# Ensembl/WiggleTools

Measured on AMD Instinct MI355X. Metric: genomic bp/s (whole node) for 'mean' over N BigWig tracks, higher is better.
Workload: dtype f64

## Files before the change

### wiggletools_amd/csrc/wt_delta.h

```cpp
#ifndef WT_DELTA_H_
#define WT_DELTA_H_

#define WT_DELTA_K 8
#define WT_DELTA_GROUP 16
#ifndef WT_DELTA_PARK
#define WT_DELTA_PARK 1
#endif
#ifndef WT_DELTA_U
#define WT_DELTA_U 4
#endif
#define WT_DELTA_TILE (64 * WT_DELTA_U)
#ifndef WT_DELTA_COPY2
#define WT_DELTA_COPY2 1
#endif
#ifndef WT_DELTA_ONE_TILE
#define WT_DELTA_ONE_TILE 1
#endif
#define WT_DELTA_TF 2048
#define WT_MAX_DELTA_T 1024
#define WT_DELTA_SQ_T0 768

struct WtDeltaShared {
    long long base_v;
    int32_t base_c;
    int32_t emin, emax, bad;
    unsigned long long base_qa, base_qb;
    long long base_v1;
    unsigned long long base_qa1, base_qb1;
    int32_t base_c1, risk;
};

#define WT_DELTA_QSHIFT 40

struct WtDeltaCtx {
    long long *acc;
    uint32_t *ev;
    long long *ltv;
    int32_t *ltc;
    long long *gtv;
    int32_t *gtc;
    long long *tbase;
    uint32_t *tpfx;
    uint16_t *tfirst;
    uint32_t *tdef;
    unsigned long long *qa, *qb;
    unsigned long long *ltqa, *ltqb;
    unsigned long long *gtqa, *gtqb;
    WtDeltaShared *dsh;
    int32_t np;
};

struct WtDeltaLane {
    long long pv[WT_DELTA_K];
    int32_t pc[WT_DELTA_K];
    uint32_t evmask;
    long long tv;
    int32_t tc;
    long long wv;
    int32_t wc;
    unsigned long long tqa, tqb;
    unsigned long long wqa, wqb;
};

WT_DEV void wt_delta_ctx_init(WtDeltaCtx &d, const WtParams &P, char *lds) {
    d.acc = (long long *) (lds + P.off_acc);
    d.ev = (uint32_t *) (lds + P.off_ev);
    d.ltv = (long long *) (lds + P.off_ltv);
    d.ltc = (int32_t *) (lds + P.off_ltc);
    d.gtv = (long long *) (lds + P.off_gtv);
    d.gtc = (int32_t *) (lds + P.off_gtc);
    d.tbase = (long long *) (lds + P.off_tbase);
    d.tpfx = (uint32_t *) (lds + P.off_tpfx);
    d.tfirst = (uint16_t *) (lds + P.off_tfirst);
    d.tdef = (uint32_t *) (lds + P.off_tdef);
    const int ns = P.delta_ns > 1 ? P.delta_ns : 1;
    d.np = ns * P.W;
    d.qa = (unsigned long long *) (lds + P.off_qa);
    d.qb = d.qa + d.np;
    d.ltqa = (unsigned long long *) (lds + P.off_ltq);
    d.ltqb = d.ltqa + ns * (P.W / WT_DELTA_K);
    d.gtqa = (unsigned long long *) (lds + P.off_gtq);
    d.gtqb = d.gtqa + ns * (P.W / WT_DELTA_K / WT_DELTA_GROUP);
    d.dsh = (WtDeltaShared *) (lds + P.off_dsh);
}

#ifdef WT_EMU
WT_DEV void wt_lds_add32(uint32_t *p, uint32_t v) { *p += v; }
WT_DEV void wt_lds_addi32(int32_t *p, int32_t v) { *p += v; }
WT_DEV void wt_lds_max32(int32_t *p, int32_t v) { if (v > *p) *p = v; }
#else
WT_DEV void wt_lds_add32(uint32_t *p, uint32_t v) { atomicAdd((unsigned int *) p, (unsigned int) v); }
WT_DEV void wt_lds_addi32(int32_t *p, int32_t v) { atomicAdd(p, v); }
WT_DEV void wt_lds_max32(int32_t *p, int32_t v) { atomicMax(p, v); }
#endif

WT_DEV int wt_delta_max_span(int n_tracks) {
    int lg = 0;
    while ((1ll << lg) < (long long) n_tracks) lg++;
    return 29 - lg;
}

template <bool QQ = false, bool TT = false>
WT_DEV void wt_delta_zero(const WtParams &P, WtCtx &c, WtDeltaCtx &d, int tid, int nt) {
    const int np = TT ? 2 * P.W : P.W;
    for (int x = tid; x < np; x += nt) { d.acc[x] = 0; d.ev[x] = 0; }
    if constexpr (QQ)
        for (int x = tid; x < np; x += nt) { d.qa[x] = 0; d.qb[x] = 0; }
    if (tid == 0) {
        d.dsh->base_v = 0; d.dsh->base_c = 0;
        if constexpr (QQ) { d.dsh->base_qa = 0; d.dsh->base_qb = 0; }
        if constexpr (TT) { d.dsh->base_v1 = 0; d.dsh->base_c1 = 0; d.dsh->base_qa1 = 0; d.dsh->base_qb1 = 0; d.dsh->risk = 0; }
        d.dsh->emin = P.def_emin; d.dsh->emax = P.def_emax; d.dsh->bad = 0;
// ... 899 lines not shown
        const unsigned higher = k + 1 < WT_DELTA_K ? um >> (k + 1) : 0u;
        const uint32_t fin_rel = higher ? (uint32_t) (p0 + k + 1 + wt_ctz64((uint64_t) higher)) : after_rel;
        sv[WT_STAGE_AT(idx)] = L.res[k];
        sp[WT_STAGE_AT(idx)] = (uint32_t) (p0 + k) | (fin_rel << 16);
        idx++;
    }
}

#ifndef WT_EMU
template <int OP>
WT_DEV void wt_delta_stage_ep(const WtParams &P, WtCtx &c, WtDeltaCtx &d, const WtLane<WT_DELTA_K> &L, unsigned em, unsigned um, unsigned idx, int tid, int nt) {
    const int per = nt / WT_BAD_SUB;
    if (c.sh->bad_slot >= 0 && tid % per == 0) c.epfx[32 + tid / per] = idx;
    if (!em) return;
    const int p0 = tid * WT_DELTA_K;
    const int32_t after = wt_next_breakpoint(P, c, p0 + WT_DELTA_K - 1);
    const int32_t w0 = c.sh->w0;
    const uint32_t after_rel = after < c.sh->w1 ? (uint32_t) (after - w0) : WT_DELTA_FAR;
    double *sv = (double *) d.acc;
    uint32_t *sp = d.ev;
#pragma unroll
    for (int k = 0; k < WT_DELTA_K; k++) {
        if (!((em >> k) & 1u)) continue;
        const unsigned higher = k + 1 < WT_DELTA_K ? um >> (k + 1) : 0u;
        const uint32_t fin_rel = higher ? (uint32_t) (p0 + k + 1 + wt_ctz64((uint64_t) higher)) : after_rel;
        sv[WT_STAGE_AT(idx)] = L.res[k];
        sp[WT_STAGE_AT(idx)] = (uint32_t) (p0 + k) | (fin_rel << 16);
        idx++;
    }
}
WT_DEV void wt_delta_note_offset_ep(const WtParams &P, WtCtx &c, int lane) {
    if (c.sh->bad_slot >= 0 && P.bad_goff && lane < WT_BAD_SUB)
        P.bad_goff[(long long) c.sh->bad_slot * WT_BAD_SUB + lane] = c.sh->goffset + (long long) c.epfx[32 + lane];
}
#endif

WT_DEV void wt_delta_copy_out(const WtParams &P, WtCtx &c, WtDeltaCtx &d, int tid, int nt) {
    const int n = c.sh->n_emit;
    const long long goff = c.sh->goffset;
    const int32_t w0 = c.sh->w0, far = c.sh->next_bp;
    const double *sv = (const double *) d.acc;
    const uint32_t *sp = d.ev;
    unsigned long long bp = 0;
#if !defined(WT_EMU) && WT_DELTA_COPY2
    struct __attribute__((packed, aligned(4))) I2 { int32_t x[2]; };
    struct __attribute__((packed, aligned(8))) D2 { double x[2]; };
    for (int i = 2 * tid; i < n; i += 2 * nt) {
        const unsigned a0 = WT_STAGE_AT((unsigned) i);
        const bool two = i + 1 < n;
        const uint32_t pf0 = sp[a0], pf1 = two ? sp[a0 + 1] : 0u;
        const double v0 = sv[a0], v1 = two ? sv[a0 + 1] : 0.0;
        const int32_t st0 = w0 + (int32_t) (pf0 & 0xffffu), st1 = w0 + (int32_t) (pf1 & 0xffffu);
        const int32_t fin0 = (pf0 >> 16) == WT_DELTA_FAR ? far : w0 + (int32_t) (pf0 >> 16);
        const int32_t fin1 = (pf1 >> 16) == WT_DELTA_FAR ? far : w0 + (int32_t) (pf1 >> 16);
        bp += (unsigned long long) (fin0 - st0) + (two ? (unsigned long long) (fin1 - st1) : 0ull);
        const long long o = goff + i;
        if (two && o + 1 < P.capacity) {
            I2 s2, f2; D2 d2;
            s2.x[0] = st0; s2.x[1] = st1; f2.x[0] = fin0; f2.x[1] = fin1; d2.x[0] = v0; d2.x[1] = v1;
            *(I2 *) (P.o_start + o) = s2;
            *(I2 *) (P.o_finish + o) = f2;
            *(D2 *) (P.o_value + o) = d2;
        } else if (o < P.capacity) {
            P.o_start[o] = st0; P.o_finish[o] = fin0; P.o_value[o] = v0;
        }
    }
#else
    for (int i = tid; i < n; i += nt) {
        const uint32_t pf = sp[WT_STAGE_AT((unsigned) i)];
        const int32_t st = w0 + (int32_t) (pf & 0xffffu);
        const int32_t fin = (pf >> 16) == WT_DELTA_FAR ? far : w0 + (int32_t) (pf >> 16);
        bp += (unsigned long long) (fin - st);
        const long long o = goff + i;
        if (o >= P.capacity) continue;
        P.o_start[o] = st;
        P.o_finish[o] = fin;
        P.o_value[o] = sv[WT_STAGE_AT((unsigned) i)];
    }
#endif
    bp = wt_wave_sum_u64(bp);
    if (bp && wt_wave_leader(tid & 63)) wt_lds_add64(&c.sh->bp_sum, bp);
}

WT_DEV void wt_delta_nextw(const WtParams &P, WtCtx &c, int tid, int nt) {
    for (int w = nt - 1 - tid; w < P.n_words; w += nt) {
        int x = w + 1;
        while (x < P.n_words && c.U[x] == 0) x++;
        c.nextw[w] = (int16_t) (x < P.n_words ? x : -1);
    }
}


#ifndef WT_EMU
WT_DEV unsigned wt_wave_scan_u32(unsigned v, int lane) {
    return wt_wave_scan32(v, 0u, [](uint32_t a, uint32_t b) { return a + b; });
}
WT_DEV long long wt_wave_scan_i64(long long v, int lane) { return (long long) wt_wave_scan_add64((unsigned long long) v); }

WT_DEV void wt_delta_ranges_w1(const WtParams &P, WtCtx &c, WtDeltaCtx &d, int c0, int tid, int nt, long long row, int chrom) {
    wt_delta_ranges1(P, c, d, c0, tid, nt, row, chrom);
    const int lane = tid & 63;
    const unsigned n = (unsigned) d.ltc[tid];
    const unsigned incl = wt_wave_scan_u32(n, lane);
    d.tpfx[tid] = incl - n;
    if (lane == 63) d.gtc[tid >> 6] = (int32_t) incl;
}
WT_DEV void wt_delta_ranges_w1(const WtParams &P, WtCtx &c, WtDeltaCtx &d, int c0, int tid, int nt) {
    wt_delta_ranges_w1(P, c, d, c0, tid, nt, c.sh->row, c.sh->chrom);
}

WT_DEV void wt_delta_ranges_w2(const WtParams &P, WtCtx &c, WtDeltaCtx &d, int tid, int nt, uint32_t tile_runs = WT_DELTA_TILE) {
    const int wave = tid >> 6;
    uint32_t pfx = d.tpfx[tid];
    pfx += wt_waves_before32((const uint32_t *) d.gtc, 0, wave, tid & 63);
    const uint32_t n = (uint32_t) d.ltc[tid];
    d.tpfx[tid] = pfx;
    d.tbase[tid] -= 4ll * (long long) pfx;
    if (tid == nt - 1) d.tpfx[nt] = pfx + n;
    for (uint32_t b = (pfx + tile_runs - 1) / tile_runs; b * tile_runs < pfx + n && b < WT_DELTA_TF; b++)
        d.tfirst[b] = (uint16_t) tid;
}

template <bool QQ = false>
WT_DEV void wt_delta_scan_w1(const WtParams &P, WtCtx &c, WtDeltaCtx &d, WtDeltaLane &L, int tid, int nt) {
    wt_delta_scan1<QQ>(P, c, d, L, tid, nt);
    const int lane = tid & 63;
    const long long rv = L.tv;
    const int32_t rc = L.tc;
    const long long iv = wt_wave_scan_i64(rv, lane);
    const int32_t ic = (int32_t) wt_wave_scan_u32((unsigned) rc, lane);
    L.wv = iv - rv;
    L.wc = ic - rc;
    if (lane == 63) { d.gtv[tid >> 6] = iv; d.gtc[tid >> 6] = ic; }
    if constexpr (QQ) {
        const unsigned long long ra = L.tqa, rb = L.tqb;
        const unsigned long long ia = (unsigned long long) wt_wave_scan_i64((long long) ra, lane);
        const unsigned long long ib = (unsigned long long) wt_wave_scan_i64((long long) rb, lane);
        L.wqa = ia - ra;
        L.wqb = ib - rb;
        if (lane == 63) { d.gtqa[tid >> 6] = ia; d.gtqb[tid >> 6] = ib; }
    }
}

WT_DEV void wt_delta_scan_w1_mm(const WtParams &P, WtCtx &c, WtDeltaCtx &d, int32_t &wc, int tid, int nt) {
    int32_t tc;
    wt_delta_scan1_mm(P, c, d, tc, tid, nt);
    const int lane = tid & 63;
    const int32_t ic = (int32_t) wt_wave_scan_u32((unsigned) tc, lane);
    wc = ic - tc;
    if (lane == 63) d.gtc[tid >> 6] = ic;
}

WT_DEV void wt_delta_scan_w1_tt(const WtParams &P, WtCtx &c, WtDeltaCtx &d, WtDeltaLane2 &L, int tid, int nts) {
    wt_delta_scan1_tt(P, c, d, L, tid, nts);
    const int lane = tid & 63, wave = tid >> 6;
    const long long iv = wt_wave_scan_i64(L.tv, lane);
    const int32_t ic = (int32_t) wt_wave_scan_u32((unsigned) L.tc, lane);
    const unsigned long long ia = (unsigned long long) wt_wave_scan_i64((long long) L.tqa, lane);
    const unsigned long long ib = (unsigned long long) wt_wave_scan_i64((long long) L.tqb, lane);
    L.wv = iv - L.tv;
    L.wc = ic - L.tc;
    L.wqa = ia - L.tqa;
    L.wqb = ib - L.tqb;
    if (lane == 63) { d.gtv[wave] = iv; d.gtc[wave] = ic; d.gtqa[wave] = ia; d.gtqb[wave] = ib; }
}

// ... 83 lines not shown
```

### wiggletools_amd/csrc/wt_delta_kernel.h

```cpp
#ifndef WT_DELTA_KERNEL_H_
#define WT_DELTA_KERNEL_H_

#include "wt_reduce_kernel.h"

#define WT_DELTA_SQ(OP) ((OP) == WT_OP_VAR || (OP) == WT_OP_STDDEV || (OP) == WT_OP_ENTROPY || (OP) == WT_OP_CV || (OP) == WT_OP_TTEST)
#ifndef WT_DELTA_MIN_WAVES
#define WT_DELTA_MIN_WAVES 4
#endif
#ifndef WT_DELTA_SQ_BLOCK
#define WT_DELTA_SQ_BLOCK WT_DELTA_SQ_T0
#endif
#ifndef WT_DELTA_ZERO_EARLY
#define WT_DELTA_ZERO_EARLY 1
#endif
#ifndef WT_DELTA_EARLY_PUBLISH
#define WT_DELTA_EARLY_PUBLISH 1
#endif
#ifndef WT_DELTA_BLOCK
#define WT_DELTA_BLOCK 1024
#endif
template <int OP, bool DF = false, int U = WT_DELTA_U>
WT_KERNEL(wt_delta_kernel, (WT_DELTA_SQ(OP) ? WT_DELTA_SQ_BLOCK : WT_DELTA_BLOCK, WT_DELTA_SQ(OP) ? 3 : WT_DELTA_MIN_WAVES), const WtParams P) {
    WT_LDS(wt_lds);
    WtCtx c;
    wt_ctx_init(c, P, wt_lds);
    WtDeltaCtx d;
    wt_delta_ctx_init(d, P, wt_lds);
    constexpr bool QQ = WT_DELTA_SQ(OP);
    constexpr bool TT = OP == WT_OP_TTEST;
    constexpr bool MM = OP == WT_OP_MAX || OP == WT_OP_MIN;
    constexpr bool EP = WT_DELTA_EARLY_PUBLISH && (OP == WT_OP_SUM || OP == WT_OP_MEAN);
    WT_REG(DL, WtDeltaLane);
    WT_REG(DL2, WtDeltaLane2);
    (void) DL; (void) DL2;
    WT_REG(L, WtLane<WT_DELTA_K>);
    WT_REG_INIT(ep_rank, 0, uint32_t); WT_REG_INIT(ep_em, 0, uint32_t);
    (void) ep_rank; (void) ep_em;
    WT_THREAD_IDS;
    const int nts = QQ ? P.W / WT_DELTA_K : nt;
#define WT_SCAN_LANE (!QQ || tid < nts)
    int guess = 0;
    long long k_dbg = -1;
    (void) k_dbg;
    WT_PROF_BEGIN;
    WT_DO() {
        if (tid == 0) {
            const long long k0 = (long long) wt_glb_add64(&P.counters[WT_CTR_TICKET], 1ull);
            c.sh->ticket = k0;
            if (k0 < P.n_windows) wt_phase_header(P, c, k0);
        }
    } WT_END
#if WT_DELTA_ZERO_EARLY
    if constexpr (MM) WT_DO() { wt_delta_zero_mm<OP == WT_OP_MAX>(P, c, d, tid, nt); } WT_END
    else WT_DO() { wt_delta_zero<QQ, TT>(P, c, d, tid, nt); } WT_END
#endif
    WT_SYNC;
    for (;;) {
        WT_MARK(101);
        const long long k = c.sh->ticket;
        k_dbg = k;
        if (k >= P.n_windows) break;
        const int nchunks = (P.n_tracks + nt - 1) / nt;
        auto ntr = [&](int ch) { const int r = P.n_tracks - ch * nt; return r < nt ? r : nt; };
#if !WT_DELTA_ZERO_EARLY
        if constexpr (MM) WT_DO() { wt_delta_zero_mm<OP == WT_OP_MAX>(P, c, d, tid, nt); } WT_END
        else WT_DO() { wt_delta_zero<QQ, TT>(P, c, d, tid, nt); } WT_END
#endif
        WT_TICK(0);
        WT_MARK(102);
        int scale = 1;
        if constexpr (MM) {
            for (int ch = 0; ch < nchunks; ch++) {
                WT_DO(ch) { wt_delta_ranges_w1(P, c, d, ch * nt, tid, nt); } WT_END
                WT_SYNC;
                WT_DELTA_RANGES_W2(P, c, d, tid, nt, 64u * U);
                WT_SYNC;
                WT_TICK(1);
                WT_DO() { wt_delta_pass_mm<OP == WT_OP_MAX>(P, c, d, tid, nt); } WT_END
                WT_SYNC;
                WT_TICK(3);
            }
            WT_DO(k) { if (tid == 0 && d.dsh->bad) wt_delta_mark_bad(P, c, k); } WT_END
        } else if (guess == 0) {
            for (int ch = 0; ch < nchunks; ch++) {
                WT_DO(ch) { wt_delta_ranges_w1(P, c, d, ch * nt, tid, nt); } WT_END
                WT_SYNC;
                WT_DELTA_RANGES_W2(P, c, d, tid, nt, 64u * U);
                WT_SYNC;
                WT_TICK(1);
                WT_DO() { wt_delta_pass1<U>(P, c, d, tid, nt); } WT_END
                WT_SYNC;
                WT_TICK(2);
            }
            const bool any = d.dsh->emin <= d.dsh->emax;
            const bool ok = wt_delta_verdict(P, d, scale);
            WT_DO(k, ok) { if (!ok && tid == 0) wt_delta_mark_bad(P, c, k); } WT_END
            for (int ch = 0; ch < nchunks; ch++) {
                if (nchunks > 1) {
                    WT_DO(ch) { wt_delta_ranges_w1(P, c, d, ch * nt, tid, nt); } WT_END
                    WT_SYNC;
                    WT_DELTA_RANGES_W2(P, c, d, tid, nt, 64u * U);
                    WT_SYNC;
                }
                WT_DO(scale, ok, ch) { wt_delta_pass2<QQ, DF, TT, U>(P, c, d, scale, ok, false, true, tid, nt, ntr(ch), ch * nt); } WT_END
                WT_SYNC;
                WT_TICK(3);
            }
            if (any && ok) guess = scale;
        } else {
            for (int ch = 0; ch < nchunks; ch++) {
                WT_DO(ch) { wt_delta_ranges_w1(P, c, d, ch * nt, tid, nt); } WT_END
                WT_SYNC;
                WT_DELTA_RANGES_W2(P, c, d, tid, nt, 64u * U);
                WT_SYNC;
                WT_TICK(1);
                WT_DO(guess, ch) { wt_delta_pass2<QQ, DF, TT, U>(P, c, d, guess, true, true, true, tid, nt, ntr(ch), ch * nt); } WT_END
                WT_SYNC;
                WT_TICK(3);
            }
            int lo;
            bool ok;
            scale = guess;
            if (!wt_delta_window_verdict(P, d, guess, lo, ok)) {
              if (!ok) {
                WT_DO(k) { if (tid == 0) wt_delta_mark_bad(P, c, k); } WT_END
              } else {
                WT_EMU_ONLY(R.n_redo++;)
                WT_SYNC;
                WT_DO() { wt_delta_rezero<QQ, TT>(P, c, d, tid, nt); } WT_END
                WT_SYNC;
                for (int ch = 0; ch < nchunks; ch++) {
                    if (nchunks > 1) {
                        WT_DO(ch) { wt_delta_ranges_w1(P, c, d, ch * nt, tid, nt); } WT_END
                        WT_SYNC;
                        WT_DELTA_RANGES_W2(P, c, d, tid, nt, 64u * U);
                        WT_SYNC;
                    }
                    WT_DO(lo, ok, ch) { wt_delta_pass2<QQ, DF, TT, U>(P, c, d, lo, ok, false, false, tid, nt, ntr(ch), ch * nt); } WT_END
                    WT_SYNC;
                }
                scale = lo;
                guess = lo;
              }
            }
        }
        WT_MARK(105);
        if constexpr (TT) {
            WT_DELTA_SCAN_W1_TT(if (tid < 2 * nts), P, c, d, WT_R(DL2), tid, nts);
            WT_SYNC;
            WT_MARK(107);
            WT_DO(scale) { if (tid < 2 * nts) wt_delta_scan3_tt(P, c, d, WT_R(DL2), scale, tid, nts); } WT_END
            WT_SYNC;
            WT_DO() { wt_delta_combine_tt(P, c, d, tid, nt); } WT_END
            WT_SYNC;
            WT_DO(k) { if (tid == 0 && d.dsh->risk && c.sh->bad_slot < 0) wt_delta_mark_bad(P, c, k); } WT_END
        } else if constexpr (MM) {
            WT_REG_INIT(wc_mm, 0, int32_t);
            WT_DELTA_SCAN_W1_MM(P, c, d, WT_R(wc_mm), tid, nt);
            WT_SYNC;
            WT_MARK(107);
            WT_DO() { wt_delta_scan3_mm<OP == WT_OP_MAX>(P, c, d, WT_R(wc_mm), WT_R(L), tid, nt); } WT_END
            WT_SYNC;
        } else if constexpr (EP) {
            WT_DELTA_SCAN_W1(, QQ, P, c, d, WT_R(DL), tid, nts);
            WT_SYNC;
            WT_MARK(107);
            WT_DO() { WT_R(ep_rank) = wt_delta_scan3_cov(P, c, d, WT_R(DL), WT_R(ep_em), tid, nts); } WT_END
            WT_SYNC;
        } else {
            WT_DELTA_SCAN_W1(if (WT_SCAN_LANE), QQ, P, c, d, WT_R(DL), tid, nts);
            WT_SYNC;
            WT_MARK(107);
            WT_DO(scale) { if (WT_SCAN_LANE) wt_delta_scan3<OP>(P, c, d, WT_R(DL), WT_R(L), scale, tid, nts); } WT_END
            WT_SYNC;
        }
        WT_TICK(4);
        WT_MARK(108);
        WT_REG_INIT(mine, 0, unsigned long long);
        if constexpr (EP) {
            WT_DO(k, scale) {
                const int lane_ = tid & 63;
                if (tid < 64) {
                    WT_R(mine) = wt_waves_before32(c.epfx, 0, nt >> 6, lane_);
                    WT_TICK(5);
                    if (tid == 0) wt_lookback_publish(P, c, k, WT_R(mine));
                }
                WT_R(ep_rank) += wt_waves_before32(c.epfx, 0, tid >> 6, lane_);
                wt_delta_scan3_val<OP>(P, c, d, WT_R(DL), WT_R(L), scale, tid, nts);
            } WT_END
        } else {
            WT_DO(k) {
                if (tid < 64) {
                    WT_R(mine) = wt_delta_escan_wave(P, c, tid);
                    WT_TICK(5);
                    if (tid == 0) wt_lookback_publish(P, c, k, WT_R(mine));
                }
            } WT_END
        }
        WT_DO() { wt_delta_nextw(P, c, tid, nt); } WT_END
        WT_SYNC;
        WT_MARK(110);
        WT_DO(k) {
            if (tid < 64) {
                wt_lookback_complete(P, c, k, tid, WT_R(mine));
                if constexpr (!EP) wt_delta_note_offset(P, c, tid);
            }
        } WT_END
        WT_TICK(6);
        if constexpr (TT) {
            WT_DO() { if (tid >= 64) wt_delta_tail_tt(P, d, tid - 64, nt - 64); } WT_END
            WT_SYNC;
            WT_TICK(2);
            WT_DO() { if (tid < nts) wt_delta_load_res_tt(P, d, WT_R(L), tid); } WT_END
            WT_SYNC;
        }
        if constexpr (EP) WT_DO() { wt_delta_stage_ep<OP>(P, c, d, WT_R(L), WT_R(ep_em), WT_R(DL).evmask, WT_R(ep_rank), tid, nts); } WT_END
        else WT_DO() { if (WT_SCAN_LANE) wt_delta_stage<OP>(P, c, d, WT_R(L), tid, nts); } WT_END
        WT_SYNC;
        if constexpr (EP) WT_DO() { if (tid < 64) wt_delta_note_offset_ep(P, c, tid); } WT_END
#ifdef WT_PROFILE_TAIL
        WT_TICK(2);
#endif
        WT_DO() { wt_delta_copy_out(P, c, d, tid, nt); } WT_END
        WT_SYNC;
#ifdef WT_PROFILE_TAIL
        WT_TICK(7);
#endif
        WT_MARK(111);
        WT_DO() {
            if (tid == 0) {
                wt_window_stats(P, c);
                const long long kn = (long long) wt_glb_add64(&P.counters[WT_CTR_TICKET], 1ull);
                c.sh->ticket = kn;
                if (kn < P.n_windows) wt_phase_header(P, c, kn);
            }
        } WT_END
#if WT_DELTA_ZERO_EARLY
        if constexpr (MM) WT_DO() { wt_delta_zero_mm<OP == WT_OP_MAX>(P, c, d, tid, nt); } WT_END
        else WT_DO() { wt_delta_zero<QQ, TT>(P, c, d, tid, nt); } WT_END
#endif
        WT_SYNC;
#ifdef WT_PROFILE_TAIL
        WT_TICK(0);
#else
        WT_TICK(7);
#endif
    }
    WT_PROF_END;
    WT_KERNEL_END;
}

#undef WT_SCAN_LANE

#endif
```

### wiggletools_amd/csrc/wt_engine.hip

```cpp
#include <hip/hip_runtime.h>

#include <cstdio>
#include <thread>
#include <atomic>
#include <cstring>
#include <map>
#include <mutex>
#include <string>
#include <vector>

#include "wt_host.h"
#include "wt_trackset.h"
#include "wt_core.h"
#include "wt_plan.h"
#include "wt_kernels.h"
#include "wt_devscope.h"
#include "wt_pool.h"

#ifndef WT_INDEX_UNROLL
#define WT_INDEX_UNROLL 2
#endif
#define WT_INDEX_CHUNK (256 * 4 * WT_INDEX_UNROLL)
__global__ void __launch_bounds__(256) wt_index_kernel(const WtParams P, long long total, long long span) {
    const long long dev_total = P.seg_off[(long long) P.n_chrom * P.n_tracks];
// ... 757 lines not shown
            }
            if (rp != WTAMD_ERR_INTERNAL) return rp;
        }
        ts->delta_failed_[dc] = true;
    }
    if (!wt_pick_plan(ts, op, n_set0, plan, err, s)) return wt_fail(WTAMD_ERR_ARG, err);
    return wt_reduce_plan(ts, plan, op, flags, n_set0, runs, d_tile, d_inplay, n_runs, s);
}

extern "C++" int wt_reduce_enqueue(wtamd_trackset *ts, const wtamd_reduce_desc &desc, wtamd_runs *runs, double *d_tile, uint8_t *d_inplay,
                                   hipStream_t s, bool *used_delta, int *delta_W) {
    WtPlan plan;
    std::string err;
    *used_delta = !d_tile && wt_wants_delta(ts, desc.op);
    if (*used_delta) {
        wt_make_delta_plan_for(plan, ts->n_tracks, desc.op);
        *delta_W = plan.W;
    } else if (!wt_pick_plan(ts, desc.op, desc.n_set0, plan, err, s)) {
        return wt_fail(WTAMD_ERR_ARG, err);
    }
    return wt_reduce_plan(ts, plan, desc.op, desc.flags, desc.n_set0, runs, d_tile, d_inplay, nullptr, s);
}

static int wt_reduce_plan(wtamd_trackset *ts, const WtPlan &plan, int op, uint32_t flags, int n_set0, wtamd_runs *runs,
                          double *d_tile, uint8_t *d_inplay, int64_t *n_runs, hipStream_t s) {
    if (plan.T > (plan.delta ? ((wt_op_is_var_family(op) || op == WT_OP_TTEST) ? wt_delta_sq_block : wt_delta_block) : wt_reduce_max_block)) return wt_fail(WTAMD_ERR_ARG, "workgroup size above the kernel's launch bound");
    WtWindows *w = nullptr;
    int rc = wt_get_windows(ts, plan.W, &w, s);
    if (rc != WTAMD_OK) return rc;
    if (!w->indexed) {
        rc = wt_build_index(ts, w, plan, s);
        if (rc != WTAMD_OK) return rc;
    }
    WtLaunch L;
    wt_fill_params(ts, w, plan, L.P);
    L.P.op = op; L.P.flags = flags; L.P.n_set0 = n_set0;
    L.P.capacity = runs->capacity;
    L.P.o_start = runs->start; L.P.o_finish = runs->finish; L.P.o_value = runs->value;
    L.P.chrom_run_off = runs->chrom_run_off ? runs->chrom_run_off : ts->d_chrom_run_off;
    L.P.o_tile = d_tile; L.P.o_inplay = d_inplay;
    L.T = plan.T; L.lds = plan.lds_bytes; L.stream = s; L.num_cu = ts->num_cu;
    L.gscratch = &ts->d_gscratch; L.gscratch_bytes = &ts->gscratch_bytes;
    if (op == WT_OP_MWU && !getenv("WTAMD_MWU_DEVICE_ERF")) {
        const int n1 = n_set0, n2 = ts->n_tracks - n_set0;
        if (ts->mwu_n1 != n1 || ts->mwu_n2 != n2) {
            std::vector<double> t;
            const bool have = wt_mwu_make_table(n1, n2, t);
            if (ts->d_mwu_table) { ts->mwu_retired.push_back(ts->d_mwu_table); ts->d_mwu_table = nullptr; }
            if (have) {
                WT_HIP(hipMalloc((void **) &ts->d_mwu_table, sizeof(double) * t.size()));
                WT_HIP(hipMemcpyAsync(ts->d_mwu_table, t.data(), sizeof(double) * t.size(), hipMemcpyHostToDevice, s));
                WT_HIP(hipStreamSynchronize(s));
            }
            ts->mwu_n1 = n1; ts->mwu_n2 = n2; ts->mwu_kmax = have ? (int) t.size() - 1 : 0;
        }
        L.P.mwu_table = ts->d_mwu_table;
        L.P.mwu_kmax = ts->mwu_kmax;
    }
    if (plan.delta) {
        const int64_t nwin = w->tab.n_windows > 0 ? w->tab.n_windows : 1;
        if (w->cap_bad < nwin) {
            int64_t c1 = w->cap_bad, c2 = w->cap_bad;
            bool quiet = false;
            WT_HIP(wt_grow(&w->d_bad_list, &c1, nwin, &quiet));
            WT_HIP(wt_grow(&w->d_bad_goff, &c2, nwin * WT_BAD_SUB, &quiet));
            w->cap_bad = c1 < c2 / WT_BAD_SUB ? c1 : c2 / WT_BAD_SUB;
        }
        L.P.bad_list = w->d_bad_list;
        L.P.bad_goff = w->d_bad_goff;
        wt_delta_defaults_params(ts->defaults.data(), ts->n_tracks, L.P);
    }

    const bool launches = w->tab.n_windows > 0 && ts->n_intervals > 0;
    {
        const long long n_status = launches ? (long long) w->tab.n_windows : 0;
        const long long most = std::max<long long>(std::max<long long>(n_status, WT_CTR_N), ts->n_chrom + 1);
        const unsigned blocks = (unsigned) std::min<long long>((most + 255) / 256, 1024);
        hipLaunchKernelGGL(wt_clear_kernel, dim3(blocks), dim3(256), 0, s, ts->d_counters, (int) WT_CTR_N, L.P.chrom_run_off, ts->n_chrom + 1,
                           w->d_status, n_status);
        WT_HIP(hipGetLastError());
    }
    if (launches) {
        if (plan.delta) {
            static const int force_u = getenv("WTAMD_DELTA_U") ? atoi(getenv("WTAMD_DELTA_U")) : 0;
            const double tiles_per_wave = (double) ts->n_intervals / (double) w->tab.n_windows / 256.0 / (double) std::max(1, L.T / 64);
            L.small_tiles = force_u == 2 || (force_u != 4 && tiles_per_wave < 8.0);
        }
        WT_HIP(hipEventRecord(ts->ev_r0, s));
        if (plan.delta) {
            wt_delta_launch(L, op);
        } else if (plan.walk_S) {
            L.err = wt_walk_launch(L.P, plan.regcol, L.T, L.lds, L.num_cu, L.gscratch, L.gscratch_bytes, L.stream, &L.grid);
        } else if (!wt_reduce_launch(L, op, ts->value_f64, ts->scratch_f32, plan.ppt, plan.n_chunks > 1 || plan.scratch_slab > 0, plan.regcol)) {
            return wt_fail(WTAMD_ERR_ARG, "op not dispatchable");
        }
        if (L.err != hipSuccess) return wt_fail(WTAMD_ERR_HIP, std::string("kernel launch: ") + hipGetErrorString(L.err));
        WT_HIP(hipEventRecord(ts->ev_r1, s));
        ts->have_reduce_time = true;
    }
    ts->stats.n_windows = w->tab.n_windows;
    ts->stats.window_bp = plan.W;
    ts->stats.lds_bytes = plan.lds_bytes;
    ts->stats.kernel = plan.delta ? 1 : (plan.walk_S ? (plan.walk_mwu ? 3 : 2) : 0);
    ts->stats.patched_windows = 0;
    if (n_runs) {
        WT_HIP(hipMemcpyAsync(ts->h_counters, ts->d_counters, sizeof(unsigned long long) * WT_CTR_N, hipMemcpyDeviceToHost, s));
        const int rcw = wt_bounded_wait([s] { return hipStreamQuery(s); }, "hipStreamQuery", nullptr, 0.002, 200, [ts](double limit_s) {
            char buf[320];
            snprintf(buf, sizeof buf, "kernel did not finish within %.0f s (debug marker %llu, window %lld; per wave %llu %llu %llu %llu %llu %llu %llu %llu)",
                     limit_s, ts->h_debug[0], (long long) ts->h_debug[1], ts->h_debug[2], ts->h_debug[3], ts->h_debug[4],
                     ts->h_debug[5], ts->h_debug[6], ts->h_debug[7], ts->h_debug[8], ts->h_debug[9]);
            return std::string(buf);
        });
        if (rcw != WTAMD_OK) return rcw;
        ts->stats.n_runs = (int64_t) ts->h_counters[WT_CTR_RUNS];
        ts->stats.covered_bp = (int64_t) ts->h_counters[WT_CTR_BP];
        ts->stats.n_intervals = (int64_t) ts->h_counters[WT_CTR_INTERVALS];
        *n_runs = ts->stats.n_runs;
        if (plan.walk_S) {
            static const bool show = getenv("WTAMD_WALK_PROF") != nullptr;
            if (show) {
                static const char *names_w[8] = {"zero+ranges", "count", "offsets", "scatter", "events", "first-median", "moves", "rest"};
                unsigned long long tot = 0;
                for (int q = 0; q < 8; q++) tot += ts->h_counters[WT_CTR_PROF + q];
                fprintf(stderr, "[wt_walk_profile]");
                for (int q = 0; q < 8; q++) fprintf(stderr, " %s %.1f%%", names_w[q], tot ? 100.0 * ts->h_counters[WT_CTR_PROF + q] / tot : 0.0);
                fprintf(stderr, " (total %.3g cycles)\n", (double) tot);
            }
        }
#ifdef WT_PROFILE
        {
            static const char *names_g[8] = {"zero", "load", "count", "emask+escan", "eval", "lookback", "write", "-"};
            static const char *names_d[8] = {"zero", "ranges", "pass1", "pass2", "scan", "escan", "lookback", "write"};
            const char **names = plan.delta ? names_d : names_g;
            unsigned long long tot = 0;
            for (int q = 0; q < 8; q++) tot += ts->h_counters[WT_CTR_PROF + q];
            fprintf(stderr, "[wt_profile] op %d:", op);
            for (int q = 0; q < 8; q++)
                fprintf(stderr, " %s %.1f%%", names[q], tot ? 100.0 * ts->h_counters[WT_CTR_PROF + q] / tot : 0.0);
            fprintf(stderr, " (total %.3g cycles over all workgroups)\n", (double) tot);
            unsigned long long p2[8] = {0};
            if (wt_prof2_take(p2))
                fprintf(stderr, "[wt_profile] register column, cycles summed over waves: gather %.3g  sort/park %.3g  count loop %.3g  erf %.3g  median sort+select %.3g\n",
                        (double) p2[0], (double) p2[1], (double) p2[2], (double) p2[3], (double) p2[4]);
        }
#endif
        if (ts->h_counters[WT_CTR_ERROR] & WT_ERR_LOOKBACK) return wt_fail(WTAMD_ERR_INTERNAL, "look-back timed out");
        if (ts->h_counters[WT_CTR_ERROR] & WT_ERR_CAPACITY) return wt_fail(WTAMD_ERR_CAPACITY, "output capacity too small");
    }
    return WTAMD_OK;
}

int wtamd_reduce(wtamd_trackset *ts, const wtamd_reduce_desc *desc, wtamd_runs *runs, int64_t *n_runs, void *stream) {
    int rc = wt_check_desc(ts, desc);
    if (rc != WTAMD_OK) return rc;
    return wt_reduce_impl(ts, desc->op, desc->flags, desc->n_set0, runs, nullptr, nullptr, n_runs, (hipStream_t) stream);
}

static int wt_reduce_host_impl(wtamd_trackset *ts, int op, uint32_t flags, int n_set0, wtamd_runs *runs,
                               double *h_tile, uint8_t *h_inplay, int64_t *n_runs) {
    if (!runs) return wt_fail(WTAMD_ERR_ARG, "runs == NULL");
    int64_t cap = wtamd_trackset_max_runs(ts);
    if (cap > runs->capacity) cap = runs->capacity;
    const int64_t alloc = cap > 0 ? cap : 1;
    const int N = ts->n_tracks;
    WtDevScope scope;
    wtamd_runs d{};
    d.capacity = cap;
    double *d_tile = nullptr;
    uint8_t *d_inplay = nullptr;
    WT_HIP(scope.alloc(&d.start, sizeof(int32_t) * alloc));
    WT_HIP(scope.alloc(&d.finish, sizeof(int32_t) * alloc));
    WT_HIP(scope.alloc(&d.value, sizeof(double) * alloc));
    WT_HIP(scope.alloc(&d.chrom_run_off, sizeof(int64_t) * (ts->n_chrom + 1)));
    if (op == WT_OP_MULTIPLEX) {
        WT_HIP(scope.alloc(&d_tile, sizeof(double) * alloc * N));
        WT_HIP(scope.alloc(&d_inplay, sizeof(uint8_t) * alloc * N));
    }
    int64_t n = 0;
    int rc = wt_reduce_impl(ts, op, flags, n_set0, &d, d_tile, d_inplay, &n, nullptr);
    if (rc == WTAMD_OK) {
        if (n > 0) {
            WT_HIP(hipMemcpy(runs->start, d.start, sizeof(int32_t) * n, hipMemcpyDeviceToHost));
            WT_HIP(hipMemcpy(runs->finish, d.finish, sizeof(int32_t) * n, hipMemcpyDeviceToHost));
            if (runs->value) WT_HIP(hipMemcpy(runs->value, d.value, sizeof(double) * n, hipMemcpyDeviceToHost));
            if (h_tile) WT_HIP(hipMemcpy(h_tile, d_tile, sizeof(double) * n * N, hipMemcpyDeviceToHost));
            if (h_inplay) WT_HIP(hipMemcpy(h_inplay, d_inplay, sizeof(uint8_t) * n * N, hipMemcpyDeviceToHost));
        }
        if (runs->chrom_run_off)
            WT_HIP(hipMemcpy(runs->chrom_run_off, d.chrom_run_off, sizeof(int64_t) * (ts->n_chrom + 1), hipMemcpyDeviceToHost));
        if (n_runs) *n_runs = n;
    }
    return rc;
}

int wtamd_reduce_host(wtamd_trackset *ts, const wtamd_reduce_desc *desc, wtamd_runs *runs, int64_t *n_runs) {
    int rc = wt_check_desc(ts, desc);
    if (rc != WTAMD_OK) return rc;
    return wt_reduce_host_impl(ts, desc->op, desc->flags, desc->n_set0, runs, nullptr, nullptr, n_runs);
}

int wtamd_multiplex_host(wtamd_trackset *ts, uint32_t flags, wtamd_runs *runs, double *values, uint8_t *inplay,
                         int64_t *n_runs) {
    if (!ts || !values || !inplay) return wt_fail(WTAMD_ERR_ARG, "NULL argument");
    return wt_reduce_host_impl(ts, WT_OP_MULTIPLEX, flags, 0, runs, values, inplay, n_runs);
}

static int wt_runs_auc_span(const wtamd_runs *runs, int64_t n_runs, double *auc, double *span, void *stream) {
    hipStream_t s = (hipStream_t) stream;
    const int blocks = 512;
    double *d_partial = nullptr, h[2] = {0, 0};
    WtDevScope scope;
    WT_HIP(scope.alloc(&d_partial, wt_auc_partial_bytes(blocks) + sizeof(double) * 2));
    const int rc = wt_auc_async(runs->start, runs->finish, runs->value, (long long) n_runs, nullptr, blocks, d_partial, d_partial + 2 * blocks, span != nullptr, s);
    if (rc != WTAMD_OK) return rc;
    WT_HIP(hipMemcpyAsync(h, d_partial + 2 * blocks, sizeof(double) * (span ? 2 : 1), hipMemcpyDeviceToHost, s));
    WT_HIP(hipStreamSynchronize(s));
// ... 99 lines not shown
```

Before: 50.62 billion.

## Drain staged output to registers and overlap lookback with clearing for sum/mean

For sum/mean with large tiles, staging now happens before the decoupled lookback completes. Each thread drains its staged (position, value) records into registers and clears the LDS accumulators while wave 0 finishes the lookback. The global stores then run after the offset is known, using paired 8/16-byte writes, and they overlap with the next window's ticket and header. This removes a barrier-separated copy-out and zero phase from the critical path, at the cost of more registers per thread for the drain buffer, which could reduce occupancy.

```diff
diff --git a/wiggletools_amd/csrc/wt_delta.h b/wiggletools_amd/csrc/wt_delta.h
--- a/wiggletools_amd/csrc/wt_delta.h
+++ b/wiggletools_amd/csrc/wt_delta.h
@@ -28,6 +28,7 @@
     long long base_v1;
     unsigned long long base_qa1, base_qb1;
     int32_t base_c1, risk;
+    long long goff;
 };
 
 #define WT_DELTA_QSHIFT 40
@@ -1093,6 +1094,86 @@
     if (bp && wt_wave_leader(tid & 63)) wt_lds_add64(&c.sh->bp_sum, bp);
 }
 
+struct WtDeltaDrain {
+    uint32_t pf[WT_DELTA_K];
+    double v[WT_DELTA_K];
+    int32_t w0, far, n;
+};
+WT_DEV void wt_delta_drain(const WtParams &P, WtCtx &c, WtDeltaCtx &d, WtDeltaDrain &R, int tid, int nt) {
+    const int n = wt_uniform32(c.sh->n_emit);
+    const int32_t w0 = wt_uniform32(c.sh->w0), far = wt_uniform32(c.sh->next_bp);
+    const double *sv = (const double *) d.acc;
+    const uint32_t *sp = d.ev;
+    unsigned long long bp = 0;
+    R.w0 = w0; R.far = far; R.n = n;
+#pragma unroll
+    for (int j = 0; j < WT_DELTA_K / 2; j++) {
+        const int i = 2 * tid + 2 * nt * j;
+        const unsigned a0 = WT_STAGE_AT((unsigned) i);
+        uint32_t pf0 = 0u, pf1 = 0u;
+        double v0 = 0.0, v1 = 0.0;
+        if (i < n) {
+            pf0 = sp[a0]; v0 = sv[a0];
+            bp += (unsigned long long) (((pf0 >> 16) == WT_DELTA_FAR ? far - w0 : (int32_t) (pf0 >> 16)) - (int32_t) (pf0 & 0xffffu));
+        }
+        if (i + 1 < n) {
+            pf1 = sp[a0 + 1]; v1 = sv[a0 + 1];
+            bp += (unsigned long long) (((pf1 >> 16) == WT_DELTA_FAR ? far - w0 : (int32_t) (pf1 >> 16)) - (int32_t) (pf1 & 0xffffu));
+        }
+        R.pf[2 * j] = pf0; R.pf[2 * j + 1] = pf1;
+        R.v[2 * j] = v0; R.v[2 * j + 1] = v1;
+    }
+    bp = wt_wave_sum_u64(bp);
+    if (bp && wt_wave_leader(tid & 63)) wt_lds_add64(&c.sh->bp_sum, bp);
+}
+WT_DEV void wt_delta_clear(const WtParams &P, WtCtx &c, WtDeltaCtx &d, int tid, int nt) {
+    const unsigned W = (unsigned) P.W, wave = (unsigned) tid >> 6, lane = (unsigned) tid & 63u;
+#pragma unroll
+    for (int j = 0; j < WT_DELTA_K / 2; j++) {
+        const unsigned r0 = 128u * wave + 2u * (unsigned) nt * (unsigned) j;
+        const unsigned a = WT_STAGE_AT(r0), e = WT_STAGE_AT(r0 + 128u);
+        const unsigned b = e < W ? e : W;
+        for (unsigned x = a + lane; x < b; x += 64u) { d.acc[x] = 0; d.ev[x] = 0; }
+    }
+    if (tid == 0) {
+        d.dsh->base_v = 0; d.dsh->base_c = 0;
+        d.dsh->emin = P.def_emin; d.dsh->emax = P.def_emax; d.dsh->bad = 0;
+    }
+}
+WT_DEV void wt_delta_store(const WtParams &P, const WtDeltaDrain &R, long long goff, int tid, int nt) {
+    const int n = R.n;
+    const int32_t w0 = R.w0, far = R.far;
+#if !defined(WT_EMU) && WT_DELTA_COPY2
+    struct __attribute__((packed, aligned(4))) I2 { int32_t x[2]; };
+    struct __attribute__((packed, aligned(8))) D2 { double x[2]; };
+#endif
+#pragma unroll
+    for (int j = 0; j < WT_DELTA_K / 2; j++) {
+        const int i = 2 * tid + 2 * nt * j;
+        if (i >= n) break;
+        const bool two = i + 1 < n;
+        const uint32_t pf0 = R.pf[2 * j], pf1 = R.pf[2 * j + 1];
+        const int32_t st0 = w0 + (int32_t) (pf0 & 0xffffu), st1 = w0 + (int32_t) (pf1 & 0xffffu);
+        const int32_t fin0 = (pf0 >> 16) == WT_DELTA_FAR ? far : w0 + (int32_t) (pf0 >> 16);
+        const int32_t fin1 = (pf1 >> 16) == WT_DELTA_FAR ? far : w0 + (int32_t) (pf1 >> 16);
+        const long long o = goff + i;
+#if !defined(WT_EMU) && WT_DELTA_COPY2
+        if (two && o + 1 < P.capacity) {
+            I2 s2, f2; D2 d2;
+            s2.x[0] = st0; s2.x[1] = st1; f2.x[0] = fin0; f2.x[1] = fin1; d2.x[0] = R.v[2 * j]; d2.x[1] = R.v[2 * j + 1];
+            *(I2 *) (P.o_start + o) = s2;
+            *(I2 *) (P.o_finish + o) = f2;
+            *(D2 *) (P.o_value + o) = d2;
+        } else if (o < P.capacity) {
+            P.o_start[o] = st0; P.o_finish[o] = fin0; P.o_value[o] = R.v[2 * j];
+        }
+#else
+        if (o < P.capacity) { P.o_start[o] = st0; P.o_finish[o] = fin0; P.o_value[o] = R.v[2 * j]; }
+        if (two && o + 1 < P.capacity) { P.o_start[o + 1] = st1; P.o_finish[o + 1] = fin1; P.o_value[o + 1] = R.v[2 * j + 1]; }
+#endif
+    }
+}
+
 WT_DEV void wt_delta_nextw(const WtParams &P, WtCtx &c, int tid, int nt) {
     for (int w = nt - 1 - tid; w < P.n_words; w += nt) {
         int x = w + 1;
diff --git a/wiggletools_amd/csrc/wt_delta_kernel.h b/wiggletools_amd/csrc/wt_delta_kernel.h
--- a/wiggletools_amd/csrc/wt_delta_kernel.h
+++ b/wiggletools_amd/csrc/wt_delta_kernel.h
@@ -36,6 +36,9 @@
     WT_REG(L, WtLane<WT_DELTA_K>);
     WT_REG_INIT(ep_rank, 0, uint32_t); WT_REG_INIT(ep_em, 0, uint32_t);
     (void) ep_rank; (void) ep_em;
+    constexpr bool DT = (OP == WT_OP_SUM || OP == WT_OP_MEAN) && U > 2 && !DF;
+    WT_REG(DR, WtDeltaDrain);
+    (void) DR;
     WT_THREAD_IDS;
     const int nts = QQ ? P.W / WT_DELTA_K : nt;
 #define WT_SCAN_LANE (!QQ || tid < nts)
@@ -200,51 +203,91 @@
         WT_DO() { wt_delta_nextw(P, c, tid, nt); } WT_END
         WT_SYNC;
         WT_MARK(110);
-        WT_DO(k) {
-            if (tid < 64) {
-                wt_lookback_complete(P, c, k, tid, WT_R(mine));
-                if constexpr (!EP) wt_delta_note_offset(P, c, tid);
-            }
-        } WT_END
-        WT_TICK(6);
-        if constexpr (TT) {
-            WT_DO() { if (tid >= 64) wt_delta_tail_tt(P, d, tid - 64, nt - 64); } WT_END
-            WT_SYNC;
+        if constexpr (DT) {
+            if constexpr (EP) WT_DO() { wt_delta_stage_ep<OP>(P, c, d, WT_R(L), WT_R(ep_em), WT_R(DL).evmask, WT_R(ep_rank), tid, nts); } WT_END
+            else WT_DO() { wt_delta_stage<OP>(P, c, d, WT_R(L), tid, nts); } WT_END
+            WT_SYNC;
+#ifdef WT_PROFILE_TAIL
             WT_TICK(2);
-            WT_DO() { if (tid < nts) wt_delta_load_res_tt(P, d, WT_R(L), tid); } WT_END
-            WT_SYNC;
-        }
-        if constexpr (EP) WT_DO() { wt_delta_stage_ep<OP>(P, c, d, WT_R(L), WT_R(ep_em), WT_R(DL).evmask, WT_R(ep_rank), tid, nts); } WT_END
-        else WT_DO() { if (WT_SCAN_LANE) wt_delta_stage<OP>(P, c, d, WT_R(L), tid, nts); } WT_END
-        WT_SYNC;
-        if constexpr (EP) WT_DO() { if (tid < 64) wt_delta_note_offset_ep(P, c, tid); } WT_END
-#ifdef WT_PROFILE_TAIL
-        WT_TICK(2);
-#endif
-        WT_DO() { wt_delta_copy_out(P, c, d, tid, nt); } WT_END
-        WT_SYNC;
-#ifdef WT_PROFILE_TAIL
-        WT_TICK(7);
-#endif
-        WT_MARK(111);
-        WT_DO() {
-            if (tid == 0) {
-                wt_window_stats(P, c);
-                const long long kn = (long long) wt_glb_add64(&P.counters[WT_CTR_TICKET], 1ull);
-                c.sh->ticket = kn;
-                if (kn < P.n_windows) wt_phase_header(P, c, kn);
-            }
-        } WT_END
+#endif
+            WT_DO() { wt_delta_drain(P, c, d, WT_R(DR), tid, nt); } WT_END
+            WT_DO(k) {
+                wt_delta_clear(P, c, d, tid, nt);
+                if (tid < 64) {
+#ifdef WT_PROFILE_TAIL
+                    WT_TICK(7);
+#endif
+                    wt_lookback_complete(P, c, k, tid, WT_R(mine));
+                    if constexpr (EP) wt_delta_note_offset_ep(P, c, tid);
+                    else wt_delta_note_offset(P, c, tid);
+                    if (tid == 0) d.dsh->goff = c.sh->goffset;
+                }
+            } WT_END
+            WT_SYNC;
+            WT_TICK(6);
+            WT_MARK(111);
+            WT_DO() { wt_delta_store(P, WT_R(DR), d.dsh->goff, tid, nt); } WT_END
+            WT_DO() {
+                if (tid == 0) {
+                    wt_window_stats(P, c);
+                    const long long kn = (long long) wt_glb_add64(&P.counters[WT_CTR_TICKET], 1ull);
+                    c.sh->ticket = kn;
+                    if (kn < P.n_windows) wt_phase_header(P, c, kn);
+                }
+            } WT_END
+            WT_SYNC;
+#ifdef WT_PROFILE_TAIL
+            WT_TICK(0);
+#else
+            WT_TICK(7);
+#endif
+        } else {
+            WT_DO(k) {
+                if (tid < 64) {
+                    wt_lookback_complete(P, c, k, tid, WT_R(mine));
+                    if constexpr (!EP) wt_delta_note_offset(P, c, tid);
+                }
+            } WT_END
+            WT_TICK(6);
+            if constexpr (TT) {
+                WT_DO() { if (tid >= 64) wt_delta_tail_tt(P, d, tid - 64, nt - 64); } WT_END
+                WT_SYNC;
+                WT_TICK(2);
+                WT_DO() { if (tid < nts) wt_delta_load_res_tt(P, d, WT_R(L), tid); } WT_END
+                WT_SYNC;
+            }
+            if constexpr (EP) WT_DO() { wt_delta_stage_ep<OP>(P, c, d, WT_R(L), WT_R(ep_em), WT_R(DL).evmask, WT_R(ep_rank), tid, nts); } WT_END
+            else WT_DO() { if (WT_SCAN_LANE) wt_delta_stage<OP>(P, c, d, WT_R(L), tid, nts); } WT_END
+            WT_SYNC;
+            if constexpr (EP) WT_DO() { if (tid < 64) wt_delta_note_offset_ep(P, c, tid); } WT_END
+#ifdef WT_PROFILE_TAIL
+            WT_TICK(2);
+#endif
+            WT_DO() { wt_delta_copy_out(P, c, d, tid, nt); } WT_END
+            WT_SYNC;
+#ifdef WT_PROFILE_TAIL
+            WT_TICK(7);
+#endif
+            WT_MARK(111);
+            WT_DO() {
+                if (tid == 0) {
+                    wt_window_stats(P, c);
+                    const long long kn = (long long) wt_glb_add64(&P.counters[WT_CTR_TICKET], 1ull);
+                    c.sh->ticket = kn;
+                    if (kn < P.n_windows) wt_phase_header(P, c, kn);
+                }
+            } WT_END
 #if WT_DELTA_ZERO_EARLY
-        if constexpr (MM) WT_DO() { wt_delta_zero_mm<OP == WT_OP_MAX>(P, c, d, tid, nt); } WT_END
-        else WT_DO() { wt_delta_zero<QQ, TT>(P, c, d, tid, nt); } WT_END
-#endif
-        WT_SYNC;
-#ifdef WT_PROFILE_TAIL
-        WT_TICK(0);
+            if constexpr (MM) WT_DO() { wt_delta_zero_mm<OP == WT_OP_MAX>(P, c, d, tid, nt); } WT_END
+            else WT_DO() { wt_delta_zero<QQ, TT>(P, c, d, tid, nt); } WT_END
+#endif
+            WT_SYNC;
+#ifdef WT_PROFILE_TAIL
+            WT_TICK(0);
 #else
-        WT_TICK(7);
-#endif
+            WT_TICK(7);
+#endif
+        }
     }
     WT_PROF_END;
     WT_KERNEL_END;
diff --git a/wiggletools_amd/csrc/wt_engine.hip b/wiggletools_amd/csrc/wt_engine.hip
--- a/wiggletools_amd/csrc/wt_engine.hip
+++ b/wiggletools_amd/csrc/wt_engine.hip
@@ -863,7 +863,8 @@
     }
     if (launches) {
         if (plan.delta) {
-            static const int force_u = getenv("WTAMD_DELTA_U") ? atoi(getenv("WTAMD_DELTA_U")) : 0;
+            const char *eu = getenv("WTAMD_DELTA_U");
+            const int force_u = eu ? atoi(eu) : 0;
             const double tiles_per_wave = (double) ts->n_intervals / (double) w->tab.n_windows / 256.0 / (double) std::max(1, L.T / 64);
             L.small_tiles = force_u == 2 || (force_u != 4 && tiles_per_wave < 8.0);
         }
@@ -912,8 +913,14 @@
 #ifdef WT_PROFILE
         {
             static const char *names_g[8] = {"zero", "load", "count", "emask+escan", "eval", "lookback", "write", "-"};
+#ifdef WT_PROFILE_TAIL
+            static const char *names_dt[8] = {"ticket+header+zero", "ranges", "staging", "pass2", "scan", "escan", "lookback", "copy-out"};
+            static const char *names_dd[8] = {"stores|ticket+header", "ranges", "staging", "pass2", "scan", "escan", "lookback-rest", "drain+clear"};
+            const char **names = !plan.delta ? names_g : ((op == WT_OP_SUM || op == WT_OP_MEAN) && !L.small_tiles) ? names_dd : names_dt;
+#else
             static const char *names_d[8] = {"zero", "ranges", "pass1", "pass2", "scan", "escan", "lookback", "write"};
             const char **names = plan.delta ? names_d : names_g;
+#endif
             unsigned long long tot = 0;
             for (int q = 0; q < 8; q++) tot += ts->h_counters[WT_CTR_PROF + q];
             fprintf(stderr, "[wt_profile] op %d:", op);
```

New measurement: 50.37 billion. About the same (-0.5%).
